# zhengchen1999/DOVE

Hardware: AMD Instinct MI355X
Metric: SR frames/s (33x720x1280 4x one-step, whole job) (higher is better)
Workload: dtype bf16; 1 GPU; synthetic 33x720x1280 HR clip (LR 180x320, 4x), one-step t=399, CogVideoX1.5-5B VAE + 42-layer DiT random-init, 1 clip per GPU (BASELINE configs[1]); weight_sums=True, vae_streams=2, variant=headline (bf16)

## Files before the change

### dove_amd/lib.py

```python
from __future__ import annotations

import ctypes as C
import os

import torch

_HERE = os.path.dirname(os.path.abspath(__file__))
LIB_PATH = os.path.join(_HERE, "libdove_hip.so")
_lib = None

F32, BF16, U8 = 0, 1, 2
METRIC_PSNR, METRIC_SSIM, METRIC_RGB_TO_Y = 1, 2, 4
COLORFIX_WAVELET, COLORFIX_ADAIN, COLORFIX_CLAMP = 1, 2, 1
YUV_444, YUV_422, YUV_420, YUV_MONO = 0, 1, 2, 3
YUV_SITING_LEFT, YUV_SITING_CENTRE = 0, 1
VIDEO_RGB_U8, VIDEO_YUV = 0, 1
RESIZE_BILINEAR, RESIZE_BICUBIC, RESIZE_AREA = 0, 1, 2
ACT_NONE, ACT_RELU, ACT_SIGMOID, ACT_TANH = 0, 1, 2, 3


class ConvDesc(C.Structure):
    _fields_ = [
        ("struct_size", C.c_uint), ("reserved", C.c_uint),
        ("x", C.c_void_p), ("cache", C.c_void_p), ("w", C.c_void_p), ("bias", C.c_void_p),
# ... 105 lines not shown

_VP, _I, _LL, _F = C.c_void_p, C.c_int, C.c_longlong, C.c_float
_ULL, _PI, _PLL = C.c_ulonglong, C.POINTER(C.c_int), C.POINTER(C.c_longlong)
XFER_FN = C.CFUNCTYPE(C.c_int, C.c_void_p, C.c_int, C.c_void_p, C.c_size_t, C.c_void_p)
GROUP_FN = C.CFUNCTYPE(C.c_int, C.c_void_p, C.c_void_p)

SIGNATURES = {
    "dove_conv_igemm_bf16": [C.POINTER(ConvDesc), _VP],
    "dove_groupnorm_stats_bf16": [_VP, _LL, _LL, _I, _F, _VP, _I, _VP, _VP],
    "dove_groupnorm_finalize_partials": [_VP, _LL, C.c_double, _F, _VP, _VP, _VP],
    "dove_groupnorm_stats_nb_bf16": [_VP, _I, _LL, _LL, _I, _F, _VP, _I, _VP, _VP],
    "dove_groupnorm_finalize_partials_nb": [_VP, _LL, _I, C.c_double, _F, _VP, C.c_size_t, _VP, _VP],
    "dove_groupnorm_apply_nb_bf16": [_VP, _VP, _I, _I, _I, _I, _I, _VP, _VP, _VP, _I, _VP, _I, _I, _I, _I, C.POINTER(C.c_int), _VP],
    "dove_avgpool_time_nb_bf16": [_VP, _I, _I, _LL, _VP, _VP],
    "dove_groupnorm_sums_bf16": [_VP, _LL, _LL, _I, _VP, _I, _VP, _VP],
    "dove_groupnorm_finalize_sums": [_VP, C.c_double, _F, _VP, _VP],
    "dove_groupnorm_sums_from_partials": [_VP, _LL, _VP, _VP, _VP],
    "dove_groupnorm_apply_bf16": [_VP, _VP, _I, _I, _I, _I, _VP, _VP, _VP, _I, _VP, _I, _I, _I, C.POINTER(C.c_int), _VP],
    "dove_layernorm_modulate_bf16": [_VP, _VP, _LL, _I, _F, _VP, _VP, _VP, _LL, _VP],
    "dove_qkv_post_bf16": [_VP, _LL, _LL, _I, _I, _I, _VP, _VP, _VP, _VP, _VP, _VP, _F, _F, _VP, _VP, _VP, _I, _VP, _VP],
    "dove_vt_quad_swap_bf16": [_VP, _LL, _LL, _VP],
    "dove_ulysses_place_bf16": [_VP, _VP, _VP, C.POINTER(C.c_longlong), _I, _I, _LL, _LL, _VP, _VP, _VP, _VP, _VP],
    "dove_cl_im2col3x3_from_ncthw": [_VP, _I, _I, _I, _I, _I, _I, _F, _F, _VP, _VP],
    "dove_conv_out_gather": [_VP, _LL, _I, _I, _I, _I, _VP, _F, _F, _F, _F, _VP, _I, _VP],
    "dove_attention_fwd_bf16": [_VP, _VP, _VP, _VP, _LL, _LL, _I, _I, _LL, _VP, _VP],
    "dove_qkv_post_mxfp8": [_VP, _LL, _LL, _I, _I, _I, _VP, _VP, _VP, _VP, _VP, _VP, _F, _F, _VP, _VP, _VP, _VP, _VP],
    "dove_attention_fwd_mxfp8": [_VP, _VP, _VP, _VP, _VP, _LL, _LL, _I, _I, _LL, _VP],
    "dove_cl_from_ncthw": [_VP, _I, _I, _LL, _I, _F, _F, _VP, _VP],
    "dove_ncthw_from_cl": [_VP, _LL, _I, _LL, _F, _F, _F, _F, _VP, _I, _VP],
    "dove_avgpool_time_bf16": [_VP, _I, _LL, _VP, _VP],
    "dove_posterior_sample": [_VP, _LL, _I, _LL, _VP, _I, _VP, _I, _VP],
    "dove_axpby": [_VP, _VP, _VP, _I, _LL, _F, _F, _VP],
    "dove_patchify": [_VP, _I, _I, _I, _I, _I, _I, _I, _VP, _LL, _VP],
    "dove_unpatchify": [_VP, _LL, _I, _I, _I, _I, _I, _I, _VP, _I, _VP],
    "dove_gemv_bf16": [_VP, _VP, _VP, _I, _I, _I, _VP, _VP],
    "dove_blend_edge_bf16": [_VP, _VP, _I, _I, _I, _I, _I, _I, _I, _I, _VP],
    "dove_preprocess_u8": [_VP, _I, _I, _I, _I, _I, _I, _I, _VP, _I, _VP],
    "dove_postprocess_u8": [_VP, _I, _I, _I, _I, _I, _I, _I, _VP, _VP],
    "dove_rmsnorm_bf16": [_VP, _VP, _LL, _I, _F, _VP, _VP],
    "dove_gated_gelu_bf16": [_VP, _VP, _LL, _I, _VP],
    "dove_attention_bias_bf16": [_VP, _VP, _VP, _LL, _VP, _VP, _LL, _I, _I, _I, _VP],
    "dove_mx_quant_bf16": [_VP, _LL, _I, _VP, _VP, _VP],
    "dove_create": [_I, C.POINTER(ModelConfig), C.POINTER(_VP)],
    "dove_set_weight": [_VP, C.c_char_p, _VP, C.POINTER(C.c_longlong), _I, _I],
    "dove_finalize_weights": [_VP],
    "dove_set_workspace": [_VP, _VP, C.c_size_t],
# ... 184 lines not shown
```

### dove_amd/ops.py

```python
from __future__ import annotations

import ctypes as C
import math
from dataclasses import dataclass

import torch

from . import lib as L


def _ru(x: int, m: int) -> int:
    return (x + m - 1) // m * m


@dataclass
class PackedConv:
    w: torch.Tensor
    bias: torch.Tensor | None
    kt: int
    kh: int
    kw: int
    cin: int
    cin_pad: int
    cout: int
# ... 369 lines not shown
def qkv_post_mx(qkv, N, Npad, heads, text_len, gq, bq, gk, bk, cos, sin, qscale, eps, Q8, K8, V8t, Vs):
    L.require_cuda(qkv, gq, bq, gk, bk, cos, sin, Q8, K8, V8t, Vs)
    L.check(L.load().dove_qkv_post_mxfp8(L.ptr(qkv), N, Npad, heads, 64, text_len, L.ptr(gq), L.ptr(bq), L.ptr(gk), L.ptr(bk),
                                         L.ptr(cos), L.ptr(sin), qscale, eps, L.ptr(Q8), L.ptr(K8), L.ptr(V8t), L.ptr(Vs),
                                         L.stream_ptr()), "dove_qkv_post_mxfp8")


def attention_mx(Q8, K8, V8t, Vs, N, Npad, heads, out):
    L.require_cuda(Q8, K8, V8t, Vs, out)
    L.check(L.load().dove_attention_fwd_mxfp8(L.ptr(Q8), L.ptr(K8), L.ptr(V8t), L.ptr(Vs), L.ptr(out), N, Npad, heads, 64,
                                              out.shape[1], L.stream_ptr()), "dove_attention_fwd_mxfp8")
    return out


def cl_im2col3x3_from_ncthw(x: torch.Tensor, cp: int, scale=1.0, shift=0.0) -> torch.Tensor:
    L.require_cuda(x)
    Cc, T, H, W = x.shape
    y = torch.empty(T, H, W, cp, dtype=torch.bfloat16, device=x.device)
    L.check(L.load().dove_cl_im2col3x3_from_ncthw(L.ptr(x), L.dt_code(x), Cc, T, H, W, cp, scale, shift, L.ptr(y), L.stream_ptr()),
            "dove_cl_im2col3x3_from_ncthw")
    return y


def conv_out_gather(p: torch.Tensor, Cc: int, bias, dtype, scale=1.0, shift=0.0, lo=-math.inf, hi=math.inf) -> torch.Tensor:
    L.require_cuda(p, bias)
    assert p.dtype == torch.float32 and p.dim() == 4
    T, H, W, ld = p.shape
    y = torch.empty(Cc, T, H, W, dtype=dtype, device=p.device)
    L.check(L.load().dove_conv_out_gather(L.ptr(p), ld, T, H, W, Cc, L.ptr(bias), scale, shift, lo, hi, L.ptr(y), L.dt_code(y),
                                          L.stream_ptr()), "dove_conv_out_gather")
    return y


def conv_out_gather_cl(p: torch.Tensor, Cc: int, bias, ld: int = 8) -> torch.Tensor:
    L.require_cuda(p, bias)
    assert p.dtype == torch.float32 and p.dim() == 4
    T, H, W, ldp = p.shape
    y = torch.empty(T, H, W, ld, dtype=torch.bfloat16, device=p.device)
    L.check(L.load().dove_conv_out_gather_cl(L.ptr(p), ldp, T, H, W, Cc, L.ptr(bias), L.ptr(y), ld, L.stream_ptr()), "dove_conv_out_gather_cl")
    return y


def tile_gather(x: torch.Tensor, t0: int, nt: int, th: int, tw: int, origins, im2col_cin: int = 0) -> torch.Tensor:
    import ctypes as C
    L.require_cuda(x)
    assert x.dtype == torch.bfloat16 and x.dim() == 4
# ... 940 lines not shown
```

### dove_amd/vae.py

```python
from __future__ import annotations

import math
import re

import torch

from . import ops
from .config import AttrDict


def frame_batches(num_frames: int, batch: int):
    n = max(num_frames // batch, 1)
    rem = num_frames % batch
    return [(batch * i + (0 if i == 0 else rem), min(batch * (i + 1) + rem, num_frames)) for i in range(n)]


def spatial_norm_tmap(t_f: int, t_z: int):
    if t_f > 1 and t_f % 2 == 1:
        if t_z == 1:
            return [0] * t_f
        return [0] + [1 + ((t - 1) * (t_z - 1)) // (t_f - 1) for t in range(1, t_f)]
    return [(t * t_z) // t_f for t in range(t_f)]


class DiagonalGaussianDistribution:

    def __init__(self, moments_cl, latent_channels, dtype):
        self._m = moments_cl
        self._L = latent_channels
        self._dtype = dtype

# ... 91 lines not shown
        if self._conv_out_split:
            w27 = w.float().permute(3, 4, 0, 1, 2).reshape(kh * kw * co, ci, kt, 1, 1)
            self.pc["decoder.conv_out.taps"] = ops.pack_conv(w27, None, dev)
            self.conv_out_bias = sd["decoder.conv_out.conv.bias"].to(dev, torch.float32).contiguous()

    def enable_slicing(self):
        self.use_slicing = True

    def disable_slicing(self):
        self.use_slicing = False

    def enable_tiling(self, *a, **k):
        self.use_tiling = True

    def disable_tiling(self):
        self.use_tiling = False

    def to(self, *a, **k):
        return self

    def _cconv(self, x, name, cache, **kw):
        pc = self.pc[name]
        kw["weight_sums"] = self.weight_sums
        nb = self._nb
        if pc.kt == 1:
            return ops.conv(x, pc, nb=nb, **kw)
        k = pc.kt - 1
        x5 = x.view(nb, x.shape[0] // nb, *x.shape[1:])
        fetch = getattr(cache, "fetch", None)
        if fetch:
            assert nb == 1, "tiles are not batched under the halo exchange"
            prev = fetch(name, (k,) + tuple(x.shape[1:]), x.device)
            prev, pair = (None if prev is None else prev[None]), True
        else:
            prev, pair = cache.get(name, (None, False))
        events = getattr(cache, "events", None)
        if events is not None and name in events:
            cache.stream.wait_event(events[name])
            prev.record_stream(cache.stream)
        tdup = kw.get("tdup", 0)
        if tdup == 1 and prev is not None and not pair:
            kw["tdup"] = 0
        if x5.shape[1] >= k:
            new = x5[:, -k:]
        else:
            pad = prev if prev is not None else x5[:, :1].expand(-1, k, -1, -1, -1)
            new = torch.cat([pad, x5], dim=1)[:, -k:].contiguous()
        if events is not None:
            events[name] = torch.cuda.Event()
            events[name].record(cache.stream)
        if fetch:
            cache.publish(name, new[0])
        else:
            cache[name] = (new, bool(tdup) and x5.shape[1] >= k)
        if prev is not None and nb == 1:
            prev = prev[0]
        return ops.conv(x, pc, cache=prev, nb=nb, **kw)

    _gn_hook = None
    _piece_role = None
    _nb = 1

    def _norm_silu(self, x, name, zq=None):
        nb = self._nb
        if self._gn_hook is not None:
            stats = self._gn_hook(x)
        else:
            stats = ops.groupnorm_stats_of(x, self.eps, nb)
        g, b = self.aff[name]
        if zq is None:
            return ops.groupnorm_apply(x, stats, g, b, silu=True, nb=nb)
        yb = ops.conv(zq, self.pc[name + ".yb"])
        ratio = x.shape[1] // zq.shape[1]
        assert x.shape[1] == zq.shape[1] * ratio and x.shape[2] == zq.shape[2] * ratio and ratio & (ratio - 1) == 0
        return ops.groupnorm_apply(x, stats, g, b, silu=True, yb=yb, sshift=ratio.bit_length() - 1,
                                   tmap=spatial_norm_tmap(x.shape[0] // nb, zq.shape[0] // nb), nb=nb)

    def _resnet(self, x, name, cache, zq=None, tdup=0):
        h = self._norm_silu(x, name + ".norm1", zq)
        h = self._cconv(h, name + ".conv1", cache, gn_eps=self.eps, tdup=tdup)
        h = self._norm_silu(h, name + ".norm2", zq)
        if name + ".conv_shortcut" in self.pc:
            x = ops.conv(x, self.pc[name + ".conv_shortcut"])
        return self._cconv(h, name + ".conv2", cache, resid=x, gn_eps=self.eps)

    def _downsample(self, x, name, compress_time):
        if compress_time:
            x = ops.avgpool_time(x, self._nb)
        return ops.conv(x, self.pc[name], stride=2, pad=(0, 0), nb=self._nb)

    def _upsample(self, x, name, compress_time):
        T = x.shape[0] // self._nb
        if compress_time and self._piece_role is not None:
            tmode, t_out = (2, 2 * T - 1) if self._piece_role == "head" else (1, 2 * T)
        elif compress_time and T > 1:
            tmode, t_out = (2, 2 * T - 1) if T % 2 == 1 else (1, 2 * T)
        else:
            tmode, t_out = 0, T
        return ops.conv(x, self.pc[name], up=1, tmode=tmode, t_out=t_out, pad=(1, 1), gn_eps=self.eps, nb=self._nb,
                        weight_sums=self.weight_sums), tmode

    def _encoder(self, x, cache, split_in=False):
        h = self._cconv(x, "encoder.conv_in.taps" if split_in and self._conv_in_split else "encoder.conv_in", cache)
        nb = len(self.boc)
        for i in range(nb):
            for j in range(self.layers):
                h = self._resnet(h, f"encoder.down_blocks.{i}.resnets.{j}", cache)
            if i < nb - 1:
                h = self._downsample(h, f"encoder.down_blocks.{i}.downsamplers.0", i < self.n_tdown)
        for j in range(2):
            h = self._resnet(h, f"encoder.mid_block.resnets.{j}", cache)
        h = self._norm_silu(h, "encoder.norm_out")
        return self._cconv(h, "encoder.conv_out", cache)

    def _decoder(self, z, cache, split_out=False):
        h = self._cconv(z, "decoder.conv_in", cache)
        for j in range(2):
            h = self._resnet(h, f"decoder.mid_block.resnets.{j}", cache, zq=z)
        nb = len(self.boc)
        tdup = 0
        for i in range(nb):
            for j in range(self.layers + 1):
                h = self._resnet(h, f"decoder.up_blocks.{i}.resnets.{j}", cache, zq=z, tdup=tdup if j == 0 else 0)
            if i < nb - 1:
                h, tdup = self._upsample(h, f"decoder.up_blocks.{i}.upsamplers.0", i < self.n_tdown)
        h = self._norm_silu(h, "decoder.norm_out", zq=z)
        if split_out and self._conv_out_split:
            return self._cconv(h, "decoder.conv_out.taps", cache, out_f32=True)
        return self._cconv(h, "decoder.conv_out", cache)

    def _tiling_params(self):
        c = self.config
        down = 2 ** (len(self.boc) - 1)
        smin_h, smin_w = c.get("sample_height", 480) // 2, c.get("sample_width", 720) // 2
        return dict(smin_h=smin_h, smin_w=smin_w, lmin_h=int(smin_h / down), lmin_w=int(smin_w / down), of_h=1 / 6, of_w=1 / 5)

    def _tiled(self, x_cl, tile_h, tile_w, stride_h, stride_w, blend_h, blend_w, lim_h, lim_w, batch, fn, im2col_cin=0):
        T, H, W, _ = x_cl.shape
        ii, jj = list(range(0, H, stride_h)), list(range(0, W, stride_w))
        rows = [[None] * len(jj) for _ in ii]
        if self.tile_batching:
            classes = {}
            for a, i in enumerate(ii):
                for b, j in enumerate(jj):
                    classes.setdefault((min(tile_h, H - i), min(tile_w, W - j)), []).append((a, b))
            split = {}
            for (shape, members) in classes.items():
                for k in range(0, len(members), self.tile_batch_max):
                    split[shape + (k,)] = members[k:k + self.tile_batch_max]
# ... 69 lines not shown
                out_row.append(tile[:, :lim_h, :lim_w])
            out_rows.append(torch.cat(out_row, dim=2))
        return torch.cat(out_rows, dim=1).contiguous()

    def _tiled_encode(self, x_cl, im2col_cin=0):
        p = self._tiling_params()
        st_h, st_w = int(p["smin_h"] * (1 - p["of_h"])), int(p["smin_w"] * (1 - p["of_w"]))
        bl_h, bl_w = int(p["lmin_h"] * p["of_h"]), int(p["lmin_w"] * p["of_w"])
        fn = (lambda xb, cache: self._encoder(xb, cache, split_in=True)) if im2col_cin else self._encoder
        return self._tiled(x_cl, p["smin_h"], p["smin_w"], st_h, st_w, bl_h, bl_w, p["lmin_h"] - bl_h, p["lmin_w"] - bl_w,
                           self.enc_batch, fn, im2col_cin)

    def _tiled_decode(self, z_cl):
        p = self._tiling_params()
        st_h, st_w = int(p["lmin_h"] * (1 - p["of_h"])), int(p["lmin_w"] * (1 - p["of_w"]))
        bl_h, bl_w = int(p["smin_h"] * p["of_h"]), int(p["smin_w"] * p["of_w"])
        fn = self._decoder
        if self._conv_out_split:
            cout, bias = self.config["out_channels"], self.conv_out_bias
            fn = lambda zb, cache: ops.conv_out_gather_cl(self._decoder(zb, cache, split_out=True), cout, bias, 8)
        return self._tiled(z_cl, p["lmin_h"], p["lmin_w"], st_h, st_w, bl_h, bl_w, p["smin_h"] - bl_h, p["smin_w"] - bl_w,
                           self.dec_batch, fn)

    def _run_batches(self, x_cl, batch, fn, post=None):
        batches = frame_batches(x_cl.shape[0], batch)
        if self.n_streams < 2 or len(batches) < 2 or not x_cl.is_cuda:
            cache, outs = {}, []
            for s, e in batches:
                o = fn(x_cl[s:e], cache)
                outs.append(post(o) if post else o)
            return outs
        if self._streams is None or len(self._streams) != self.n_streams:
            self._streams = [torch.cuda.Stream(device=self.device) for _ in range(self.n_streams)]
        main = torch.cuda.current_stream(self.device)
        cache, outs = StreamCache(), []
        for st in self._streams:
            st.wait_stream(main)
        for i, (s, e) in enumerate(batches):
            st = self._streams[i % len(self._streams)]
            cache.stream = st
            with torch.cuda.stream(st):
                xb = x_cl[s:e]
                xb.record_stream(st)
                o = fn(xb, cache)
                o = post(o) if post else o
                outs.append(o)
        for st in self._streams:
            main.wait_stream(st)
        for o in outs:
            o.record_stream(main)
        return outs

    @torch.no_grad()
    def encode(self, x: torch.Tensor, return_dict: bool = True):
        if x.dim() != 5:
            raise ValueError("expected [B,C,F,H,W]")
        tp = self._tiling_params()
        tiled = self.use_tiling and (x.shape[-1] > tp["smin_w"] or x.shape[-2] > tp["smin_h"])
        x = x.to(self.device).contiguous()
        cin_pad = self.pc["encoder.conv_in"].cin_pad
        moments = []
        for b in range(x.shape[0]):
            if tiled:
                if self._conv_in_split:
                    moments.append(self._tiled_encode(ops.cl_im2col3x3_from_ncthw(x[b], self.pc["encoder.conv_in.taps"].cin_pad),
                                                      im2col_cin=x.shape[1]))
                else:
                    moments.append(self._tiled_encode(ops.cl_from_ncthw(x[b], cin_pad)))
                continue
            if self._conv_in_split:
                x_cl = ops.cl_im2col3x3_from_ncthw(x[b], self.pc["encoder.conv_in.taps"].cin_pad)
                outs = self._run_batches(x_cl, self.enc_batch, lambda xb, cache: self._encoder(xb, cache, split_in=True))
            else:
                outs = self._run_batches(ops.cl_from_ncthw(x[b], cin_pad), self.enc_batch, self._encoder)
            moments.append(torch.cat(outs, dim=0) if len(outs) > 1 else outs[0])
        dist = DiagonalGaussianDistribution(moments, self.lat, self.dtype)
        return _Out(latent_dist=dist) if return_dict else (dist,)

    @torch.no_grad()
    def decode(self, z: torch.Tensor, return_dict: bool = True, _range01: bool = False, _prescale: float = 1.0):
        z = z.to(self.device).contiguous()
        cin_pad = self.pc["decoder.conv_in"].cin_pad
        cout = self.config["out_channels"]
        post = dict(scale=0.5, shift=0.5, lo=0.0, hi=1.0) if _range01 else {}
        tp = self._tiling_params()
        tiled = self.use_tiling and (z.shape[-1] > tp["lmin_w"] or z.shape[-2] > tp["lmin_h"])
        vids = []
        for b in range(z.shape[0]):
            z_cl = ops.cl_from_ncthw(z[b], cin_pad, scale=_prescale)
            if tiled:
                vids.append(ops.ncthw_from_cl(self._tiled_decode(z_cl), cout, self.dtype, **post))
                continue
            if self._conv_out_split:
                outs = self._run_batches(z_cl, self.dec_batch, lambda zb, cache: self._decoder(zb, cache, split_out=True),
                                         post=lambda o: ops.conv_out_gather(o, cout, self.conv_out_bias, self.dtype, **post))
            else:
                outs = self._run_batches(z_cl, self.dec_batch, self._decoder, post=lambda o: ops.ncthw_from_cl(o, cout, self.dtype, **post))
            vids.append(torch.cat(outs, dim=1) if len(outs) > 1 else outs[0])
        sample = torch.stack(vids)
        return _Out(sample=sample) if return_dict else (sample,)
```

### include/dove_hip.h

```cpp
#ifndef DOVE_HIP_H
#define DOVE_HIP_H

#include <stddef.h>

#ifdef __cplusplus
extern "C" {
#endif

#define DOVE_ABI_VERSION 15

#define DOVE_F32 0
#define DOVE_BF16 1

const char* dove_last_error(void);
int dove_abi_version(void);
int dove_device_info(int dev, char* name, int name_len, int* cu_count, long long* total_mem);

typedef struct dove_conv_desc {
  unsigned int struct_size;
  unsigned int reserved;
  const void* x;
  const void* cache;
  const void* w;
  const float* bias;
// ... 41 lines not shown
int dove_avgpool_time_nb_bf16(const void* x, int nb, int T, long long frame_elems, void* y, void* stream);

int dove_layernorm_modulate_bf16(const void* x, void* y, long long rows, int D, float eps, const float* gamma,
                                 const float* beta, const float* mod, long long split, void* stream);

int dove_qkv_post_bf16(const void* qkv, long long N, long long Npad, int heads, int head_dim, int text_len,
                       const float* gq, const float* bq, const float* gk, const float* bk, const float* cosT,
                       const float* sinT, float qscale, float eps, void* Qh, void* Kh, void* Vt, int v_order, float* norm2, void* stream);
int dove_vt_quad_swap_bf16(void* Vt, long long rows, long long Npad, void* stream);
int dove_ulysses_place_bf16(const void* rq, const void* rk, const void* rv, const long long* counts, int world, int hloc, long long N,
                            long long Npad, void* Qh, void* Kh, void* Vt, float* norm2_out, void* stream);

int dove_attention_fwd_bf16(const void* Qh, const void* Kh, const void* Vt, void* O, long long N, long long Npad,
                            int heads, int head_dim, long long ldo, float* norm2, void* stream);
int dove_attention_head_paths(const float* norm2_host, int heads, int* path);
const char* dove_attention_path_name(int path);

int dove_cl_from_ncthw(const void* x, int dtype, int C, long long npix, int Cp, float scale, float shift, void* y,
                       void* stream);
int dove_ncthw_from_cl(const void* x, long long ld, int C, long long npix, float scale, float shift, float lo,
                       float hi, void* y, int dtype, void* stream);
int dove_cl_im2col3x3_from_ncthw(const void* x, int dtype, int C, int T, int H, int W, int Cp, float scale, float shift, void* y,
                                 void* stream);
int dove_conv_out_gather(const float* p, long long ldp, int T, int H, int W, int C, const float* bias, float scale, float shift, float lo,
                         float hi, void* y, int dtype, void* stream);
int dove_avgpool_time_bf16(const void* x, int T, long long frame_elems, void* y, void* stream);
int dove_posterior_sample(const void* moments, long long ld, int latent_channels, long long npix, const void* noise,
                          int noise_dtype, void* out, int out_dtype, void* stream);
int dove_axpby(const void* x, const void* y, void* out, int dtype, long long n, float a, float b, void* stream);
int dove_patchify(const void* x, int dtype, int T, int C, int H, int W, int pt, int p, void* tokens, long long ld,
                  void* stream);
int dove_unpatchify(const void* tokens, long long ld, int T, int C, int H, int W, int pt, int p, void* y, int dtype,
                    void* stream);
int dove_conv_out_gather_cl(const float* p, long long ldp, int T, int H, int W, int C, const float* bias, void* y, int ldy, void* stream);
int dove_tile_gather_bf16(const void* x, int H, int W, int C, int t0, int nt, int th, int tw, int nb, const int* oy, const int* ox,
                          int im2col_cin, void* out, void* stream);
int dove_blend_edge_bf16(const void* a, void* b, int T, int Ha, int Wa, int Hb, int Wb, int ld, int extent, int axis,
                         void* stream);
int dove_preprocess_u8(const void* frames, int F0, int H0, int W0, int pad_f, int pad_h, int pad_w, int upscale, void* out,
                       int out_dtype, void* stream);
int dove_postprocess_u8(const void* video, int dtype, int F, int H, int W, int Fo, int Ho, int Wo, void* out, void* stream);

#define DOVE_U8 2
#define DOVE_METRIC_PSNR 1
#define DOVE_METRIC_SSIM 2
#define DOVE_METRIC_RGB_TO_Y 4
typedef struct dove_image_view {
  const void* data;
// ... 297 lines not shown
```

Before: 35.06 frames/s.

## Fuse VAE encoder conv_in and decoder conv_out ends into dedicated MFMA kernels

Adds a fused encoder conv_in kernel that reads the 3-channel NCTHW input directly, builds the im2col slab in LDS and applies the causal temporal taps with a ring buffer. This removes the separate im2col materialisation pass. It also adds a fused decoder conv_out kernel that does the 3-tap temporal reduction and the spatial gather, bias and clamp in one pass instead of writing f32 partials and gathering them afterwards. A dedicated pointwise kernel handles large shortcut 1x1 convs. The new kernels are specialised to fixed channel counts and take on extra correctness risk in halo and cache handling.

```diff
diff --git a/dove_amd/csrc/vae_ends.hip b/dove_amd/csrc/vae_ends.hip
--- /dev/null
+++ b/dove_amd/csrc/vae_ends.hip
@@ -0,0 +1,456 @@
+#include "common.h"
+#include "../../include/dove_hip.h"
+
+namespace vae_ends {
+constexpr int CI_BM = 128;
+constexpr int CI_C = 3;
+constexpr int CI_CP = 32;
+constexpr int CI_CO = 128;
+constexpr int CI_SLAB = CI_BM * CI_CP * 2;
+constexpr int CI_RING = 4;
+constexpr int CI_TR = 32 * CI_CO * 2;
+constexpr int CI_LDS = CI_RING * CI_SLAB + 4 * CI_TR + CI_CO * 4;
+
+struct ConvInArgs {
+  const void* x;
+  const void* cache;
+  const bf16_t* w;
+  const float* bias;
+  bf16_t* out;
+  long long sx_c, sx_t, sc_c, sc_t;
+  int T, H, W, tiles_w;
+  float scale, shift;
+};
+
+__device__ __forceinline__ float ld_elem(const void* p, long long i, bool f32) {
+  return f32 ? ((const float*)p)[i] : bf2f(((const bf16_t*)p)[i]);
+}
+}
+
+template <bool kF32>
+__global__ __launch_bounds__(256, 2) void conv_in_fused_kernel(const vae_ends::ConvInArgs a) {
+  using namespace vae_ends;
+  extern __shared__ __attribute__((aligned(16))) char smem[];
+  const int tid = threadIdx.x, lane = tid & 63;
+  const int wave = __builtin_amdgcn_readfirstlane(tid >> 6);
+  const int h = blockIdx.x / a.tiles_w, ow0 = (blockIdx.x - h * a.tiles_w) * CI_BM;
+
+  const int m = tid & (CI_BM - 1), half = tid >> 7;
+  const int ow = ow0 + m;
+  unsigned inmask = 0;
+  int poff[16];
+#pragma unroll
+  for (int e = 0; e < 16; ++e) {
+    const int k = half * 16 + e, tap = k / CI_C, c = k - tap * CI_C;
+    const int dy = tap / 3 - 1, dx = tap % 3 - 1;
+    const bool in = tap < 9 && h + dy >= 0 && h + dy < a.H && ow + dx >= 0 && ow + dx < a.W;
+    inmask |= (in ? 1u : 0u) << e;
+    poff[e] = (h + dy) * a.W + ow + dx;
+  }
+  const int sw = (m >> 2) & 3;
+  char* const slab_w0 = smem + m * 64 + (((2 * half) ^ sw) * 16);
+  char* const slab_w1 = smem + m * 64 + (((2 * half + 1) ^ sw) * 16);
+
+  float raw[16];
+  auto fetch = [&](int fv) {
+    const void* base;
+    long long sc;
+    if (fv >= 0) { base = (const char*)a.x + fv * a.sx_t * (kF32 ? 4 : 2); sc = a.sx_c; }
+    else if (a.cache) { base = (const char*)a.cache + (2 + fv) * a.sc_t * (kF32 ? 4 : 2); sc = a.sc_c; }
+    else { base = a.x; sc = a.sx_c; }
+#pragma unroll
+    for (int e = 0; e < 16; ++e)
+      raw[e] = ld_elem(base, ((inmask >> e) & 1u) ? ((half * 16 + e) % CI_C) * sc + poff[e] : 0ll, kF32);
+  };
+  auto build = [&](int slot) {
+    float f[16];
+#pragma unroll
+    for (int e = 0; e < 16; ++e) f[e] = ((inmask >> e) & 1u) ? raw[e] * a.scale + a.shift : 0.f;
+    *(uint4*)(slab_w0 + slot * CI_SLAB) = pack8(f);
+    *(uint4*)(slab_w1 + slot * CI_SLAB) = pack8(f + 8);
+  };
+
+  const int hi = lane >> 5, l31 = lane & 31;
+  const int prow = wave * 32 + l31;
+  int xoff[2];
+#pragma unroll
+  for (int kk = 0; kk < 2; ++kk) xoff[kk] = prow * 64 + (((kk * 2 + hi) ^ ((prow >> 2) & 3)) * 16);
+  bf16x8 wf[3][2][4];
+#pragma unroll
+  for (int dt = 0; dt < 3; ++dt)
+#pragma unroll
+    for (int kk = 0; kk < 2; ++kk)
+#pragma unroll
+      for (int i = 0; i < 4; ++i)
+        wf[dt][kk][i] = *(const bf16x8*)(a.w + ((long long)(dt * CI_CO + i * 32 + l31) * CI_CP + (kk * 2 + hi) * 8));
+
+  char* const tr = smem + CI_RING * CI_SLAB + wave * CI_TR;
+  const int tr_w = l31 * 256, tr_sw = l31 & 15;
+  const int sp = lane >> 4, sq = lane & 15;
+
+  float* const bias_s = (float*)(smem + CI_RING * CI_SLAB + 4 * CI_TR);
+  if (a.bias && tid < CI_CO) bias_s[tid] = a.bias[tid];
+
+  fetch(-2); build(2);
+  fetch(-1); build(3);
+  fetch(0);
+  for (int tl = 0; tl < a.T; ++tl) {
+    build(tl & 3);
+    if (tl + 1 < a.T) fetch(tl + 1);
+    __syncthreads();
+    f32x16 acc[4];
+#pragma unroll
+    for (int i = 0; i < 4; ++i)
+#pragma unroll
+      for (int r = 0; r < 16; ++r) acc[i][r] = 0.f;
+#pragma unroll
+    for (int dt = 0; dt < 3; ++dt) {
+      const char* slab = smem + ((tl + dt + 2) & 3) * CI_SLAB;
+#pragma unroll
+      for (int kk = 0; kk < 2; ++kk) {
+        const bf16x8 xf = *(const bf16x8*)(slab + xoff[kk]);
+#pragma unroll
+        for (int i = 0; i < 4; ++i) acc[i] = __builtin_amdgcn_mfma_f32_32x32x16_bf16(wf[dt][kk][i], xf, acc[i], 0, 0, 0);
+      }
+    }
+#pragma unroll
+    for (int i = 0; i < 4; ++i)
+#pragma unroll
+      for (int g = 0; g < 4; ++g) {
+        const int cb = i * 32 + 8 * g + 4 * hi;
+        float v[4];
+#pragma unroll
+        for (int e = 0; e < 4; ++e) v[e] = acc[i][g * 4 + e];
+        if (a.bias) {
+          const f32x4 b = *(const f32x4*)(bias_s + cb);
+#pragma unroll
+          for (int e = 0; e < 4; ++e) v[e] += b[e];
+        }
+        uint2 o;
+        o.x = pack_bf2(v[0], v[1]);
+        o.y = pack_bf2(v[2], v[3]);
+        *(uint2*)(tr + tr_w + ((((cb * 2) >> 4) ^ tr_sw) * 16) + ((cb * 2) & 15)) = o;
+      }
+    bf16_t* const orow = a.out + (((long long)tl * a.H + h) * a.W + ow0 + wave * 32) * CI_CO;
+#pragma unroll
+    for (int r = 0; r < 8; ++r) {
+      const int px = 4 * r + sp;
+      const uint4 v = *(const uint4*)(tr + px * 256 + ((sq ^ (px & 15)) * 16));
+      if (ow0 + wave * 32 + px < a.W) *(uint4*)(orow + (long long)px * CI_CO + sq * 8) = v;
+    }
+  }
+}
+
+extern "C" int dove_conv_in_fused(const void* x, int dtype, long long sx_c, long long sx_t, const void* cache, long long sc_c, long long sc_t,
+                                  int C, int T, int H, int W, float scale, float shift, const void* w, int cin_pad, int cout_pad,
+                                  const float* bias, void* out, void* stream) {
+  using namespace vae_ends;
+  DOVE_CHECK_ARG(x && w && out, "conv_in_fused: null pointer");
+  DOVE_CHECK_ARG(dtype == DOVE_F32 || dtype == DOVE_BF16, "conv_in_fused: bad dtype %d", dtype);
+  DOVE_CHECK_ARG(C == CI_C && cin_pad == CI_CP && cout_pad == CI_CO,
+                 "conv_in_fused: built for 3 input channels (27 im2col channels padded to 32) and 128 output channels (C %d, cin_pad %d, cout_pad %d)",
+                 C, cin_pad, cout_pad);
+  DOVE_CHECK_ARG(T > 0 && H > 0 && W > 0 && (long long)H * W < (1ll << 31), "conv_in_fused: bad extent %d x %d x %d", T, H, W);
+  DOVE_CHECK_ARG(sx_c >= 0 && sx_t >= 0 && (!cache || (sc_c >= 0 && sc_t >= 0)), "conv_in_fused: negative stride");
+  DOVE_CHECK_ARG(((uintptr_t)w & 15) == 0 && ((uintptr_t)out & 15) == 0 && (!bias || ((uintptr_t)bias & 15) == 0),
+                 "conv_in_fused: weights, bias and output must be 16-byte aligned");
+  ConvInArgs a;
+  a.x = x; a.cache = cache; a.w = (const bf16_t*)w; a.bias = bias; a.out = (bf16_t*)out;
+  a.sx_c = sx_c; a.sx_t = sx_t; a.sc_c = sc_c; a.sc_t = sc_t;
+  a.T = T; a.H = H; a.W = W; a.tiles_w = (W + CI_BM - 1) / CI_BM;
+  a.scale = scale; a.shift = shift;
+  const long long grid = (long long)H * a.tiles_w;
+  DOVE_CHECK_ARG(grid < (1ll << 31), "conv_in_fused: grid too large");
+  static PerDeviceOnce attr_set;
+  if (auto once_ = attr_set.guard()) {
+    (void)hipFuncSetAttribute((const void*)conv_in_fused_kernel<true>, hipFuncAttributeMaxDynamicSharedMemorySize, CI_LDS);
+    (void)hipFuncSetAttribute((const void*)conv_in_fused_kernel<false>, hipFuncAttributeMaxDynamicSharedMemorySize, CI_LDS);
+  }
+  if (dtype == DOVE_F32) hipLaunchKernelGGL(conv_in_fused_kernel<true>, dim3((unsigned)grid), dim3(256), CI_LDS, (hipStream_t)stream, a);
+  else hipLaunchKernelGGL(conv_in_fused_kernel<false>, dim3((unsigned)grid), dim3(256), CI_LDS, (hipStream_t)stream, a);
+  DOVE_CHECK_LAUNCH("dove_conv_in_fused");
+  return DOVE_OK;
+}
+
+namespace vae_ends {
+constexpr int CO_TH = 8, CO_TW = 64, CO_RW = CO_TW + 2, CO_NREC = (CO_TH + 2) * CO_RW;
+constexpr int CO_CI = 128, CO_NP = 32, CO_C = 3, CO_LREC = 9 * CO_C;
+constexpr int CO_P_BYTES = CO_NREC * CO_LREC * 4;
+constexpr int CO_W_BYTES = 3 * CO_NP * CO_CI * 2;
+constexpr int CO_LDS = CO_P_BYTES + CO_W_BYTES;
+
+struct ConvOutArgs {
+  const bf16_t* x;
+  const bf16_t* cache;
+  const bf16_t* w;
+  const float* bias;
+  void* y;
+  int dt, T, H, W, tiles_w;
+  float scale, shift, lo, hi;
+};
+}
+
+__global__ __launch_bounds__(512) void conv_out_fused_kernel(const vae_ends::ConvOutArgs a) {
+  using namespace vae_ends;
+  extern __shared__ __attribute__((aligned(16))) char smem[];
+  float* const P = (float*)smem;
+  char* const wl = smem + CO_P_BYTES;
+  const int tid = threadIdx.x, lane = tid & 63;
+  const int wave = __builtin_amdgcn_readfirstlane(tid >> 6);
+  const unsigned id = xcd_remap(blockIdx.x, gridDim.x);
+  const int ty = id / a.tiles_w, tx = id - ty * a.tiles_w;
+  const int x0 = tx * CO_TW, y0 = ty * CO_TH;
+
+#pragma unroll
+  for (int r = 0; r < 3; ++r) {
+    const int j = tid + 512 * r, row = (j >> 4) & 31, ch = j & 15;
+    *(uint4*)(wl + (j >> 9) * (CO_NP * 256) + row * 256 + ((ch ^ (row & 15)) * 16)) = *(const uint4*)(a.w + (long long)j * 8);
+  }
+
+  const int hi = lane >> 5, l31 = lane & 31;
+  int poff[3], rec[3];
+  bool inf[3];
+#pragma unroll
+  for (int b = 0; b < 3; ++b) {
+    rec[b] = (wave * 3 + b) * 32 + l31;
+    const int ry = rec[b] / CO_RW, rx = rec[b] - ry * CO_RW;
+    const int iy = y0 + ry - 1, ix = x0 + rx - 1;
+    inf[b] = rec[b] < CO_NREC && iy >= 0 && iy < a.H && ix >= 0 && ix < a.W;
+    poff[b] = (inf[b] ? (iy * a.W + ix) * (CO_CI * 2) : 0) + hi * 16;
+  }
+  const int woff = l31 * 256;
+  const int wsw = l31 & 15;
+  const long long frame_bytes = (long long)a.H * a.W * (CO_CI * 2);
+  const long long npix = (long long)a.T * a.H * a.W;
+  float bz[CO_C];
+#pragma unroll
+  for (int c = 0; c < CO_C; ++c) bz[c] = a.bias ? a.bias[c] : 0.f;
+  const int lx = tid & 63, rr = tid >> 6;
+  const int oy = y0 + rr, ox = x0 + lx;
+  const bool ovalid = oy < a.H && ox < a.W;
+
+  f32x16 accA[3], accB[3];
+#pragma unroll
+  for (int b = 0; b < 3; ++b)
+#pragma unroll
+    for (int r = 0; r < 16; ++r) { accA[b][r] = 0.f; accB[b][r] = 0.f; }
+  __syncthreads();
+
+  auto step = [&](int f, f32x16 (&O)[3], f32x16 (&M)[3]) {
+    const char* src = f >= 0 ? (const char*)a.x + f * frame_bytes : (a.cache ? (const char*)a.cache + (2 + f) * frame_bytes : (const char*)a.x);
+    auto wfrag = [&](int tap, int q) { return *(const bf16x8*)(wl + tap * (CO_NP * 256) + woff + (((q * 2 + hi) ^ wsw) * 16)); };
+    bf16x8 xf[2][8];
+#pragma unroll
+    for (int q = 0; q < 8; ++q) xf[0][q] = *(const bf16x8*)(src + poff[0] + q * 32);
+#pragma unroll
+    for (int b = 0; b < 3; ++b) {
+      if (b < 2) {
+#pragma unroll
+        for (int q = 0; q < 8; ++q) xf[(b + 1) & 1][q] = *(const bf16x8*)(src + poff[b + 1] + q * 32);
+      }
+      const bf16x8(&xb)[8] = xf[b & 1];
+      if (f >= 0) {
+#pragma unroll
+        for (int q = 0; q < 8; ++q) O[b] = __builtin_amdgcn_mfma_f32_32x32x16_bf16(wfrag(2, q), xb[q], O[b], 0, 0, 0);
+        if (rec[b] < CO_NREC) {
+#pragma unroll
+          for (int g = 0; g < 4; ++g)
+#pragma unroll
+            for (int e = 0; e < 4; ++e) {
+              const int col = 8 * g + 4 * hi + e;
+              if (col < CO_LREC) P[rec[b] * CO_LREC + col] = inf[b] ? O[b][g * 4 + e] : 0.f;
+            }
+        }
+      }
+#pragma unroll
+      for (int r = 0; r < 16; ++r) O[b][r] = 0.f;
+#pragma unroll
+      for (int q = 0; q < 8; ++q) O[b] = __builtin_amdgcn_mfma_f32_32x32x16_bf16(wfrag(0, q), xb[q], O[b], 0, 0, 0);
+#pragma unroll
+      for (int q = 0; q < 8; ++q) M[b] = __builtin_amdgcn_mfma_f32_32x32x16_bf16(wfrag(1, q), xb[q], M[b], 0, 0, 0);
+    }
+    if (f < 0) return;
+    __syncthreads();
+    if (ovalid) {
+      float acc[CO_C];
+#pragma unroll
+      for (int c = 0; c < CO_C; ++c) acc[c] = 0.f;
+#pragma unroll
+      for (int dy = 0; dy < 3; ++dy)
+#pragma unroll
+        for (int dx = 0; dx < 3; ++dx) {
+          const float* q = P + ((rr + dy) * CO_RW + lx + dx) * CO_LREC + (dy * 3 + dx) * CO_C;
+#pragma unroll
+          for (int c = 0; c < CO_C; ++c) acc[c] += q[c];
+        }
+      const long long pix = ((long long)f * a.H + oy) * a.W + ox;
+#pragma unroll
+      for (int c = 0; c < CO_C; ++c) {
+        const float v = bf2f(f2bf(acc[c] + bz[c]));
+        const float o = fminf(fmaxf(v * a.scale + a.shift, a.lo), a.hi);
+        if (a.dt == DOVE_F32) ((float*)a.y)[(long long)c * npix + pix] = o;
+        else ((bf16_t*)a.y)[(long long)c * npix + pix] = f2bf(o);
+      }
+    }
+    __syncthreads();
+  };
+
+  for (int f = -2; f < a.T; f += 2) {
+    step(f, accA, accB);
+    if (f + 1 < a.T) step(f + 1, accB, accA);
+  }
+}
+
+extern "C" int dove_conv_out_fused(const void* x, const void* cache, int T, int H, int W, int cin, const void* w, int cout_pad, int C,
+                                   const float* bias, float scale, float shift, float lo, float hi, void* y, int dtype, void* stream) {
+  using namespace vae_ends;
+  DOVE_CHECK_ARG(x && w && y, "conv_out_fused: null pointer");
+  DOVE_CHECK_ARG(dtype == DOVE_F32 || dtype == DOVE_BF16, "conv_out_fused: bad dtype %d", dtype);
+  DOVE_CHECK_ARG(cin == CO_CI && cout_pad == CO_NP && C == CO_C,
+                 "conv_out_fused: built for 128 input channels and 3 output channels (27 tap channels padded to 32); got cin %d, cout_pad %d, C %d",
+                 cin, cout_pad, C);
+  DOVE_CHECK_ARG(T > 0 && H > 0 && W > 0 && (long long)H * W * (CO_CI * 2) < (1ll << 31), "conv_out_fused: bad extent %d x %d x %d", T, H, W);
+  DOVE_CHECK_ARG(((uintptr_t)x & 15) == 0 && ((uintptr_t)w & 15) == 0 && (!cache || ((uintptr_t)cache & 15) == 0),
+                 "conv_out_fused: input, cache and weights must be 16-byte aligned");
+  ConvOutArgs a;
+  a.x = (const bf16_t*)x; a.cache = (const bf16_t*)cache; a.w = (const bf16_t*)w; a.bias = bias; a.y = y;
+  a.dt = dtype; a.T = T; a.H = H; a.W = W; a.tiles_w = (W + CO_TW - 1) / CO_TW;
+  a.scale = scale; a.shift = shift; a.lo = lo; a.hi = hi;
+  const long long grid = (long long)a.tiles_w * ((H + CO_TH - 1) / CO_TH);
+  DOVE_CHECK_ARG(grid < (1ll << 31), "conv_out_fused: grid too large");
+  static PerDeviceOnce attr_set;
+  if (auto once_ = attr_set.guard())
+    (void)hipFuncSetAttribute((const void*)conv_out_fused_kernel, hipFuncAttributeMaxDynamicSharedMemorySize, CO_LDS);
+  hipLaunchKernelGGL(conv_out_fused_kernel, dim3((unsigned)grid), dim3(512), CO_LDS, (hipStream_t)stream, a);
+  DOVE_CHECK_LAUNCH("dove_conv_out_fused");
+  return DOVE_OK;
+}
+
+namespace vae_ends {
+struct PwArgs {
+  const bf16_t* x;
+  const bf16_t* w;
+  const float* bias;
+  bf16_t* out;
+  long long M, ldo;
+  int cin, nblk;
+};
+}
+
+template <int KF, int CT>
+__global__ __launch_bounds__(512) void pointwise_conv_kernel(const vae_ends::PwArgs a) {
+  using namespace vae_ends;
+  constexpr int WCH = KF * 2, WPITCH = KF * 32 + 16;
+  constexpr int W_BYTES = CT * 32 * WPITCH;
+  constexpr int CPP = CT * 4, TROW = CT * 64, TR_BYTES = 32 * TROW;
+  extern __shared__ __attribute__((aligned(16))) char smem[];
+  char* const wl = smem;
+  const int tid = threadIdx.x, lane = tid & 63;
+  const int wave = __builtin_amdgcn_readfirstlane(tid >> 6);
+  char* const tr = smem + W_BYTES + wave * TR_BYTES;
+  float* const bias_s = (float*)(smem + W_BYTES + 8 * TR_BYTES);
+  const int n0 = blockIdx.y * (CT * 32);
+
+  for (int j = tid; j < CT * 32 * WCH; j += 512) {
+    const int row = j / WCH, ch = j - row * WCH;
+    *(uint4*)(wl + row * WPITCH + ch * 16) = *(const uint4*)(a.w + ((long long)(n0 + row) * a.cin + ch * 8));
+  }
+  if (a.bias && tid < CT * 32) bias_s[tid] = a.bias[n0 + tid];
+  __syncthreads();
+
+  const int hi = lane >> 5, l31 = lane & 31;
+  const int stride = gridDim.x * 8;
+  const char* const wfb = wl + l31 * WPITCH + hi * 16;
+  auto load = [&](bf16x8 (&xf)[KF], int b) {
+    const long long pix = (long long)b * 32 + l31;
+    const char* src = (const char*)a.x + (pix < a.M ? pix : 0) * (long long)(KF * 32) + hi * 16;
+#pragma unroll
+    for (int k = 0; k < KF; ++k) xf[k] = *(const bf16x8*)(src + k * 32);
+  };
+  bf16x8 xc[KF], xn[KF];
+  int b = blockIdx.x * 8 + wave;
+  if (b < a.nblk) load(xc, b);
+  for (; b < a.nblk; b += stride) {
+    if (b + stride < a.nblk) load(xn, b + stride);
+    f32x16 acc[CT];
+#pragma unroll
+    for (int i = 0; i < CT; ++i)
+#pragma unroll
+      for (int r = 0; r < 16; ++r) acc[i][r] = 0.f;
+#pragma unroll
+    for (int k = 0; k < KF; ++k)
+#pragma unroll
+      for (int i = 0; i < CT; ++i) {
+        const bf16x8 wf = *(const bf16x8*)(wfb + i * 32 * WPITCH + k * 32);
+        acc[i] = __builtin_amdgcn_mfma_f32_32x32x16_bf16(wf, xc[k], acc[i], 0, 0, 0);
+      }
+#pragma unroll
+    for (int i = 0; i < CT; ++i)
+#pragma unroll
+      for (int g = 0; g < 4; ++g) {
+        const int cb = i * 32 + 8 * g + 4 * hi;
+        float v[4];
+#pragma unroll
+        for (int e = 0; e < 4; ++e) v[e] = acc[i][g * 4 + e];
+        if (a.bias) {
+          const f32x4 bb = *(const f32x4*)(bias_s + cb);
+#pragma unroll
+          for (int e = 0; e < 4; ++e) v[e] += bb[e];
+        }
+        uint2 o;
+        o.x = pack_bf2(v[0], v[1]);
+        o.y = pack_bf2(v[2], v[3]);
+        *(uint2*)(tr + l31 * TROW + ((((cb * 2) >> 4) ^ (l31 & (CPP - 1))) * 16) + ((cb * 2) & 15)) = o;
+      }
+#pragma unroll
+    for (int r = 0; r < CPP / 2; ++r) {
+      const int px = r * (64 / CPP) + lane / CPP, q = lane % CPP;
+      const uint4 v = *(const uint4*)(tr + px * TROW + ((q ^ (px & (CPP - 1))) * 16));
+      const long long pix = (long long)b * 32 + px;
+      if (pix < a.M) *(uint4*)(a.out + pix * a.ldo + n0 + q * 8) = v;
+    }
+#pragma unroll
+    for (int k = 0; k < KF; ++k) xc[k] = xn[k];
+  }
+}
+
+namespace vae_ends {
+template <int KF, int CT>
+static int launch_pointwise(const PwArgs& a, int tiles_n, hipStream_t s) {
+  constexpr int lds = CT * 32 * (KF * 32 + 16) + 8 * 32 * CT * 64 + CT * 32 * 4;
+  static PerDeviceOnce attr_set;
+  if (auto once_ = attr_set.guard())
+    (void)hipFuncSetAttribute((const void*)pointwise_conv_kernel<KF, CT>, hipFuncAttributeMaxDynamicSharedMemorySize, lds);
+  int dev = 0, cus = 256;
+  (void)hipGetDevice(&dev);
+  (void)hipDeviceGetAttribute(&cus, hipDeviceAttributeMultiprocessorCount, dev);
+  const int want = (a.nblk + 7) / 8;
+  const int G = want < cus ? want : cus;
+  hipLaunchKernelGGL((pointwise_conv_kernel<KF, CT>), dim3((unsigned)G, (unsigned)tiles_n), dim3(512), lds, s, a);
+  DOVE_CHECK_LAUNCH("dove_pointwise_conv_bf16");
+  return DOVE_OK;
+}
+}
+
+extern "C" int dove_pointwise_conv_bf16(const void* x, long long M, int cin, const void* w, int cout_pad, int cout, const float* bias, void* out,
+                                        long long ldo, void* stream) {
+  using namespace vae_ends;
+  DOVE_CHECK_ARG(x && w && out, "pointwise_conv: null pointer");
+  DOVE_CHECK_ARG(cin == 64 || cin == 128 || cin == 256, "pointwise_conv: Cin must be 64, 128 or 256 (got %d)", cin);
+  DOVE_CHECK_ARG(cout > 0 && cout % 64 == 0 && cout_pad >= cout && cout_pad % 32 == 0, "pointwise_conv: Cout must be a positive multiple of 64 (got %d of %d)",
+                 cout, cout_pad);
+  DOVE_CHECK_ARG(M > 0 && (M + 31) / 32 < (1ll << 31), "pointwise_conv: bad row count %lld", M);
+  DOVE_CHECK_ARG(ldo >= cout && ldo % 8 == 0, "pointwise_conv: ldo (%lld) must be a multiple of 8 and >= Cout", ldo);
+  DOVE_CHECK_ARG(((uintptr_t)x & 15) == 0 && ((uintptr_t)w & 15) == 0 && ((uintptr_t)out & 15) == 0 && (!bias || ((uintptr_t)bias & 15) == 0),
+                 "pointwise_conv: operands must be 16-byte aligned");
+  PwArgs a;
+  a.x = (const bf16_t*)x; a.w = (const bf16_t*)w; a.bias = bias; a.out = (bf16_t*)out;
+  a.M = M; a.ldo = ldo; a.cin = cin; a.nblk = (int)((M + 31) / 32);
+  hipStream_t s = (hipStream_t)stream;
+  if (cout % 128 == 0) {
+    const int tn = cout / 128;
+    return cin == 256 ? launch_pointwise<16, 4>(a, tn, s) : (cin == 128 ? launch_pointwise<8, 4>(a, tn, s) : launch_pointwise<4, 4>(a, tn, s));
+  }
+  const int tn = cout / 64;
+  return cin == 256 ? launch_pointwise<16, 2>(a, tn, s) : (cin == 128 ? launch_pointwise<8, 2>(a, tn, s) : launch_pointwise<4, 2>(a, tn, s));
+}
diff --git a/dove_amd/lib.py b/dove_amd/lib.py
--- a/dove_amd/lib.py
+++ b/dove_amd/lib.py
@@ -151,6 +151,9 @@
     "dove_vt_quad_swap_bf16": [_VP, _LL, _LL, _VP],
     "dove_ulysses_place_bf16": [_VP, _VP, _VP, C.POINTER(C.c_longlong), _I, _I, _LL, _LL, _VP, _VP, _VP, _VP, _VP],
     "dove_cl_im2col3x3_from_ncthw": [_VP, _I, _I, _I, _I, _I, _I, _F, _F, _VP, _VP],
+    "dove_conv_in_fused": [_VP, _I, _LL, _LL, _VP, _LL, _LL, _I, _I, _I, _I, _F, _F, _VP, _I, _I, _VP, _VP, _VP],
+    "dove_conv_out_fused": [_VP, _VP, _I, _I, _I, _I, _VP, _I, _I, _VP, _F, _F, _F, _F, _VP, _I, _VP],
+    "dove_pointwise_conv_bf16": [_VP, _LL, _I, _VP, _I, _I, _VP, _VP, _LL, _VP],
     "dove_conv_out_gather": [_VP, _LL, _I, _I, _I, _I, _VP, _F, _F, _F, _F, _VP, _I, _VP],
     "dove_attention_fwd_bf16": [_VP, _VP, _VP, _VP, _LL, _LL, _I, _I, _LL, _VP, _VP],
     "dove_qkv_post_mxfp8": [_VP, _LL, _LL, _I, _I, _I, _VP, _VP, _VP, _VP, _VP, _VP, _F, _F, _VP, _VP, _VP, _VP, _VP],
diff --git a/dove_amd/ops.py b/dove_amd/ops.py
--- a/dove_amd/ops.py
+++ b/dove_amd/ops.py
@@ -415,6 +415,84 @@
     return y
 
 
+def pointwise_conv_ok(x: torch.Tensor, pc: PackedConv) -> bool:
+    return (pc.kt == 1 and pc.kh == 1 and pc.kw == 1 and pc.cin_pad == pc.cin and pc.cin in (64, 128, 256) and pc.cout % 64 == 0
+            and x.shape[-1] == pc.cin)
+
+
+def pointwise_conv(x: torch.Tensor, pc: PackedConv, *, ldo: int | None = None, out: torch.Tensor | None = None) -> torch.Tensor:
+    L.require_cuda(x, out)
+    assert x.dtype == torch.bfloat16 and pointwise_conv_ok(x, pc), (x.dtype, x.shape, pc.cin, pc.cout)
+    M = x.numel() // x.shape[-1]
+    ldo = pc.cout_store if ldo is None else ldo
+    if out is None:
+        out = torch.empty(*x.shape[:-1], ldo, dtype=torch.bfloat16, device=x.device)
+    else:
+        assert out.shape == (*x.shape[:-1], ldo) and out.dtype == torch.bfloat16
+    if _profiler is not None:
+        e0, e1 = torch.cuda.Event(enable_timing=True), torch.cuda.Event(enable_timing=True)
+        e0.record()
+    L.check(L.load().dove_pointwise_conv_bf16(L.ptr(x), M, pc.cin, L.ptr(pc.w), pc.cout_pad, pc.cout, L.ptr(pc.bias), L.ptr(out), ldo, L.stream_ptr()),
+            "dove_pointwise_conv_bf16")
+    if _profiler is not None:
+        e1.record()
+        flops = 2.0 * M * pc.cout * pc.cin
+        _profiler.append(((pc.cin, pc.cout, 1), flops, e0, e1, "pointwise_conv_kernel", flops))
+    return out
+
+
+def conv_in_fused(x: torch.Tensor, pc: PackedConv, *, cache: torch.Tensor | None = None, scale=1.0, shift=0.0, nb: int = 1,
+                  weight_sums: bool = True, out: torch.Tensor | None = None) -> torch.Tensor:
+    assert x.dim() == 4 and (cache is None or cache.dim() == 4)
+    L.require_cuda(x[0, 0], None if cache is None else cache[0, 0])
+    assert nb == 1 and pc.kt == 3 and pc.kh == 1 and pc.kw == 1, (nb, x.shape, pc.kt, pc.kh, pc.kw)
+    T, Cc, H, W = x.shape
+    assert x.stride(3) == 1 and x.stride(2) == W, x.stride()
+    if cache is not None:
+        assert cache.shape == (2, Cc, H, W) and cache.dtype == x.dtype and cache.stride(3) == 1 and cache.stride(2) == W, (cache.shape, cache.stride())
+    if out is None:
+        out = torch.empty(T, H, W, pc.cout_store, dtype=torch.bfloat16, device=x.device)
+    else:
+        L.require_cuda(out)
+        assert out.shape == (T, H, W, pc.cout_store) and out.dtype == torch.bfloat16 and out.is_contiguous()
+    if _profiler is not None:
+        e0, e1 = torch.cuda.Event(enable_timing=True), torch.cuda.Event(enable_timing=True)
+        e0.record()
+    L.check(L.load().dove_conv_in_fused(L.ptr(x), L.dt_code(x), x.stride(1), x.stride(0), L.ptr(cache), cache.stride(1) if cache is not None else 0,
+                                        cache.stride(0) if cache is not None else 0, Cc, T, H, W, scale, shift, L.ptr(pc.w), pc.cin_pad,
+                                        pc.cout_pad, L.ptr(pc.bias), L.ptr(out), L.stream_ptr()), "dove_conv_in_fused")
+    if _profiler is not None:
+        e1.record()
+        flops = 2.0 * T * H * W * pc.cout * pc.cin * pc.kt
+        _profiler.append(((pc.cin, pc.cout, pc.kt), flops, e0, e1, "conv_in_fused_kernel", flops))
+    return out
+
+
+def conv_out_fused(x: torch.Tensor, pc: PackedConv, *, Cc: int, bias, dtype, cache: torch.Tensor | None = None, scale=1.0, shift=0.0,
+                   lo=-math.inf, hi=math.inf, nb: int = 1, weight_sums: bool = True, out: torch.Tensor | None = None) -> torch.Tensor:
+    L.require_cuda(x, cache, bias, out)
+    assert nb == 1 and x.dtype == torch.bfloat16 and x.dim() == 4 and pc.kt == 3 and pc.kh == 1 and pc.kw == 1 and pc.bias is None
+    T, H, W, Cx = x.shape
+    assert pc.cout == 9 * Cc and Cx == pc.cin_pad, (pc.cout, Cc, Cx, pc.cin_pad)
+    if cache is not None:
+        assert cache.shape == (2, H, W, Cx) and cache.dtype == torch.bfloat16, (cache.shape, x.shape)
+    if out is None:
+        out = torch.empty(Cc, T, H, W, dtype=dtype, device=x.device)
+    else:
+        assert out.shape == (Cc, T, H, W) and out.dtype == dtype
+    if _profiler is not None:
+        e0, e1 = torch.cuda.Event(enable_timing=True), torch.cuda.Event(enable_timing=True)
+        e0.record()
+    L.check(L.load().dove_conv_out_fused(L.ptr(x), L.ptr(cache), T, H, W, Cx, L.ptr(pc.w), pc.cout_pad, Cc, L.ptr(bias), scale, shift, lo, hi,
+                                         L.ptr(out), L.dt_code(out), L.stream_ptr()), "dove_conv_out_fused")
+    if _profiler is not None:
+        e1.record()
+        flops = 2.0 * T * H * W * pc.cout * pc.cin * pc.kt
+        real = flops * (-(-H // 8) * -(-W // 64) * 660.0) / (H * W)
+        _profiler.append(((pc.cin, pc.cout, pc.kt), flops, e0, e1, "conv_out_fused_kernel", real))
+    return out
+
+
 def conv_out_gather(p: torch.Tensor, Cc: int, bias, dtype, scale=1.0, shift=0.0, lo=-math.inf, hi=math.inf) -> torch.Tensor:
     L.require_cuda(p, bias)
     assert p.dtype == torch.float32 and p.dim() == 4
diff --git a/dove_amd/vae.py b/dove_amd/vae.py
--- a/dove_amd/vae.py
+++ b/dove_amd/vae.py
@@ -7,6 +7,9 @@
 
 from . import ops
 from .config import AttrDict
+
+FUSED_ENDS = True
+PW_MIN_PIXELS = 900_000
 
 
 def frame_batches(num_frames: int, batch: int):
@@ -144,6 +147,7 @@
     def _cconv(self, x, name, cache, **kw):
         pc = self.pc[name]
         kw["weight_sums"] = self.weight_sums
+        conv = kw.pop("op", ops.conv)
         nb = self._nb
         if pc.kt == 1:
             return ops.conv(x, pc, nb=nb, **kw)
@@ -159,7 +163,8 @@
         events = getattr(cache, "events", None)
         if events is not None and name in events:
             cache.stream.wait_event(events[name])
-            prev.record_stream(cache.stream)
+            if prev.untyped_storage().data_ptr() != x.untyped_storage().data_ptr():
+                prev.record_stream(cache.stream)
         tdup = kw.get("tdup", 0)
         if tdup == 1 and prev is not None and not pair:
             kw["tdup"] = 0
@@ -177,10 +182,11 @@
             cache[name] = (new, bool(tdup) and x5.shape[1] >= k)
         if prev is not None and nb == 1:
             prev = prev[0]
-        return ops.conv(x, pc, cache=prev, nb=nb, **kw)
+        return conv(x, pc, cache=prev, nb=nb, **kw)
 
     _gn_hook = None
     _piece_role = None
+    _fused_pw = False
     _nb = 1
 
     def _norm_silu(self, x, name, zq=None):
@@ -203,7 +209,11 @@
         h = self._cconv(h, name + ".conv1", cache, gn_eps=self.eps, tdup=tdup)
         h = self._norm_silu(h, name + ".norm2", zq)
         if name + ".conv_shortcut" in self.pc:
-            x = ops.conv(x, self.pc[name + ".conv_shortcut"])
+            pcs = self.pc[name + ".conv_shortcut"]
+            if self._fused_pw and x.numel() // x.shape[-1] >= PW_MIN_PIXELS and pcs.cout <= 256 and ops.pointwise_conv_ok(x, pcs):
+                x = ops.pointwise_conv(x, pcs)
+            else:
+                x = ops.conv(x, pcs)
         return self._cconv(h, name + ".conv2", cache, resid=x, gn_eps=self.eps)
 
     def _downsample(self, x, name, compress_time):
@@ -222,8 +232,12 @@
         return ops.conv(x, self.pc[name], up=1, tmode=tmode, t_out=t_out, pad=(1, 1), gn_eps=self.eps, nb=self._nb,
                         weight_sums=self.weight_sums), tmode
 
-    def _encoder(self, x, cache, split_in=False):
-        h = self._cconv(x, "encoder.conv_in.taps" if split_in and self._conv_in_split else "encoder.conv_in", cache)
+    def _encoder(self, x, cache, split_in=False, fused_in=False):
+        self._fused_pw = fused_in
+        if fused_in:
+            h = self._cconv(x, "encoder.conv_in.taps", cache, op=ops.conv_in_fused)
+        else:
+            h = self._cconv(x, "encoder.conv_in.taps" if split_in and self._conv_in_split else "encoder.conv_in", cache)
         nb = len(self.boc)
         for i in range(nb):
             for j in range(self.layers):
@@ -235,7 +249,8 @@
         h = self._norm_silu(h, "encoder.norm_out")
         return self._cconv(h, "encoder.conv_out", cache)
 
-    def _decoder(self, z, cache, split_out=False):
+    def _decoder(self, z, cache, split_out=False, fused_out=None):
+        self._fused_pw = fused_out is not None
         h = self._cconv(z, "decoder.conv_in", cache)
         for j in range(2):
             h = self._resnet(h, f"decoder.mid_block.resnets.{j}", cache, zq=z)
@@ -247,6 +262,8 @@
             if i < nb - 1:
                 h, tdup = self._upsample(h, f"decoder.up_blocks.{i}.upsamplers.0", i < self.n_tdown)
         h = self._norm_silu(h, "decoder.norm_out", zq=z)
+        if fused_out is not None:
+            return self._cconv(h, "decoder.conv_out.taps", cache, op=ops.conv_out_fused, **fused_out)
         if split_out and self._conv_out_split:
             return self._cconv(h, "decoder.conv_out.taps", cache, out_f32=True)
         return self._cconv(h, "decoder.conv_out", cache)
@@ -362,7 +379,7 @@
         return self._tiled(z_cl, p["lmin_h"], p["lmin_w"], st_h, st_w, bl_h, bl_w, p["smin_h"] - bl_h, p["smin_w"] - bl_w,
                            self.dec_batch, fn)
 
-    def _run_batches(self, x_cl, batch, fn, post=None):
+    def _run_batches(self, x_cl, batch, fn, post=None, own_input=True):
         batches = frame_batches(x_cl.shape[0], batch)
         if self.n_streams < 2 or len(batches) < 2 or not x_cl.is_cuda:
             cache, outs = {}, []
@@ -381,7 +398,8 @@
             cache.stream = st
             with torch.cuda.stream(st):
                 xb = x_cl[s:e]
-                xb.record_stream(st)
+                if own_input:
+                    xb.record_stream(st)
                 o = fn(xb, cache)
                 o = post(o) if post else o
                 outs.append(o)
@@ -390,6 +408,10 @@
         for o in outs:
             o.record_stream(main)
         return outs
+
+    def _conv_in_fusable(self, x):
+        pc = self.pc["encoder.conv_in.taps"]
+        return x.shape[1] == 3 and pc.cin_pad == 32 and pc.cout_pad == 128 and pc.cout_store == 128 and x.dtype in (torch.float32, torch.bfloat16)
 
     @torch.no_grad()
     def encode(self, x: torch.Tensor, return_dict: bool = True):
@@ -408,7 +430,10 @@
                 else:
                     moments.append(self._tiled_encode(ops.cl_from_ncthw(x[b], cin_pad)))
                 continue
-            if self._conv_in_split:
+            if self._conv_in_split and FUSED_ENDS and self._conv_in_fusable(x):
+                outs = self._run_batches(x[b].permute(1, 0, 2, 3), self.enc_batch, lambda xb, cache: self._encoder(xb, cache, fused_in=True),
+                                         own_input=False)
+            elif self._conv_in_split:
                 x_cl = ops.cl_im2col3x3_from_ncthw(x[b], self.pc["encoder.conv_in.taps"].cin_pad)
                 outs = self._run_batches(x_cl, self.enc_batch, lambda xb, cache: self._encoder(xb, cache, split_in=True))
             else:
@@ -431,7 +456,11 @@
             if tiled:
                 vids.append(ops.ncthw_from_cl(self._tiled_decode(z_cl), cout, self.dtype, **post))
                 continue
-            if self._conv_out_split:
+            pct = self.pc.get("decoder.conv_out.taps")
+            if self._conv_out_split and FUSED_ENDS and pct.cin_pad == 128 and pct.cout == 27:
+                fused = dict(Cc=cout, bias=self.conv_out_bias, dtype=self.dtype, **post)
+                outs = self._run_batches(z_cl, self.dec_batch, lambda zb, cache: self._decoder(zb, cache, fused_out=fused))
+            elif self._conv_out_split:
                 outs = self._run_batches(z_cl, self.dec_batch, lambda zb, cache: self._decoder(zb, cache, split_out=True),
                                          post=lambda o: ops.conv_out_gather(o, cout, self.conv_out_bias, self.dtype, **post))
             else:
diff --git a/include/dove_hip.h b/include/dove_hip.h
--- a/include/dove_hip.h
+++ b/include/dove_hip.h
@@ -87,8 +87,15 @@
                        float hi, void* y, int dtype, void* stream);
 int dove_cl_im2col3x3_from_ncthw(const void* x, int dtype, int C, int T, int H, int W, int Cp, float scale, float shift, void* y,
                                  void* stream);
+int dove_conv_in_fused(const void* x, int dtype, long long sx_c, long long sx_t, const void* cache, long long sc_c, long long sc_t, int C,
+                       int T, int H, int W, float scale, float shift, const void* w, int cin_pad, int cout_pad, const float* bias, void* out,
+                       void* stream);
 int dove_conv_out_gather(const float* p, long long ldp, int T, int H, int W, int C, const float* bias, float scale, float shift, float lo,
                          float hi, void* y, int dtype, void* stream);
+int dove_conv_out_fused(const void* x, const void* cache, int T, int H, int W, int cin, const void* w, int cout_pad, int C, const float* bias,
+                        float scale, float shift, float lo, float hi, void* y, int dtype, void* stream);
+int dove_pointwise_conv_bf16(const void* x, long long M, int cin, const void* w, int cout_pad, int cout, const float* bias, void* out,
+                             long long ldo, void* stream);
 int dove_avgpool_time_bf16(const void* x, int T, long long frame_elems, void* y, void* stream);
 int dove_posterior_sample(const void* moments, long long ld, int latent_channels, long long npix, const void* noise,
                           int noise_dtype, void* out, int out_dtype, void* stream);
```

Result: no change. 35.38 frames/s (median of 6 runs) (+0.9%).
